# edin-dal/sdqlpy

Measured on AMD Instinct MI355X. Metric: tpch_q1_q3_q5_sf10_rows_per_sec, higher is better.
Workload: dtype f64; 1 GPU; TPCH Q1+Q3+Q5 SF=10 per GPU (BASELINE metric: Q1/Q3/Q5 at SF=10; q1 = configs[1], q3 = configs[2]); partitioning=none

## Files before the change

### sdqlpy_amd/csrc/sdqh_hip.hip

```cpp
#include <hip/hip_runtime.h>

#include <algorithm>
#include <atomic>
#include <chrono>
#include <cmath>
#include <cstdio>
#include <cstdlib>
#include <cstring>
#include <string>
#include <thread>
#include <type_traits>
#include <map>
#include <vector>

#include "sdqh_host.hpp"

using namespace sdqh_host;

static int ensure_index(sdqh_ctx* ctx, sdqh_table* tb);

namespace sdqh_host {

int fail(sdqh_ctx* ctx, int code, const std::string& msg) {
    if (ctx) ctx->err = msg;
// ... 620 lines not shown
    const std::string n(name);
    if (n == "resident_cap" && value >= 1 && value <= 8) ctx->opt_resident_cap = (int)value;
    else if (n == "async_copies" && (value == 0 || value == 1)) ctx->opt_async_copies = (int)value;
    else if (n == "resident_stream" && value >= 1 && value <= 8) ctx->opt_resident_stream = (int)value;
    else if (n == "probe_chunk" && value >= 1 && value <= 64) ctx->opt_probe_chunk = (int)value;
    else if (n == "probe_unroll" && (value == 1 || value == 2 || value == 4)) ctx->opt_probe_unroll = (int)value;
    else if (n == "stage_batch" && (value == 2 || value == 4 || value == 8)) ctx->opt_stage_batch = (int)value;
    else if (n == "stage_eager" && (value == 0 || value == 1)) ctx->opt_stage_eager = (int)value;
    else if (n == "stage_eager_pay" && (value == 0 || value == 1)) ctx->opt_stage_eager_pay = (int)value;
    else if (n == "stage_waves_per_cu" && value >= 4 && value <= 64) ctx->opt_stage_waves_per_cu = (int)value;
    else if (n == "direct_index" && (value == 0 || value == 1)) ctx->opt_direct_index = (int)value;
    else if (n == "row_pack" && (value == 0 || value == 1)) ctx->opt_row_pack = (int)value;
    else if (n == "cluster_pack" && value >= 0 && value <= 2) ctx->opt_cluster_pack = (int)value;
    else if (n == "cluster_list" && (value == 0 || value == 1)) ctx->opt_cluster_list = (int)value;
    else if (n == "x_driven" && value >= 0 && value <= (1 << 20)) ctx->opt_x_driven = (int)value;
    else if (n == "delta8" && (value == 0 || value == 1)) ctx->opt_delta8 = (int)value;
    else if (n == "word_pairs" && (value == 0 || value == 1)) ctx->opt_word_pairs = (int)value;
    else if (n == "coarse_kb" && value >= 0 && value <= 96) ctx->opt_coarse_kb = (int)value;
    else if (n == "lookup_pipeline" && value >= -1 && value <= 1) ctx->opt_lookup_pipeline = (int)value;
    else if (n == "probe_pipeline" && value >= 0 && value <= 1) ctx->opt_probe_pipeline = (int)value;
    else if (n == "lookup_debug") ctx->opt_lookup_debug = (int)value;
    else if (n == "fuse_small" && value >= 0 && value <= 1) ctx->opt_fuse_small = (int)value;
    else if (n == "lds_key_set" && value >= 0 && value <= 1) ctx->opt_lds_key_set = (int)value;
    else if (n == "fill_ahead" && value >= 0 && value <= 1) { ctx->opt_fill_ahead = (int)value; for (auto& b : ctx->pool) b.nhabits = 0; }
    else if (n == "str_rows" && (value == 0 || value == 32 || value == 64)) ctx->opt_str_rows = (int)value;
    else if (n == "rank_increasing" && value >= 0 && value <= 1) ctx->opt_rank_increasing = (int)value;
    else if (n == "feature_min_rows" && value >= 0) ctx->opt_feature_min_rows = value;
    else if (n == "narrow" && value >= 0 && value <= 1) ctx->opt_narrow = (int)value;
    else if (n == "tight" && value >= 0 && value <= 1) ctx->opt_tight = (int)value;
    else if (n == "spin_sync" && value >= 0 && value <= 1) ctx->opt_spin_sync = (int)value;
// ... 1964 lines not shown
```

### sdqlpy_amd/csrc/sdqh_host.hpp

```cpp
#pragma once
#include <hip/hip_runtime.h>

#include <atomic>
#include <map>
#include <string>
#include <vector>

#include "sdqh.h"
#include "sdqh_kernels.hpp"

namespace sdqh_host {

struct FillHabit { size_t off, bytes; int byte; bool clean; };
struct PoolBlock {
    void* ptr; size_t size; bool free;
    FillHabit habits[4] = {};
    int nhabits = 0;
    uint64_t alloc_seq = 0;
    bool fill_use = false;
    const void* graph_owner = nullptr;
};
struct ProfEntry { const char* name; hipEvent_t e0, e1; double ms; int64_t model_bytes; };

constexpr size_t STAGING_BYTES = 32u << 20;
// ... 65 lines not shown
    int opt_tight = 1;
    hipStream_t side[2] = {nullptr, nullptr};
    hipEvent_t side_ev[4] = {nullptr, nullptr, nullptr, nullptr};
    int opt_side_streams = 1;
    int opt_side_priority = 1;
    int opt_copy_kernel = 0;
    int opt_copy_nt = 1;
    int opt_row_index = 1;
    int opt_grouped_index = 1;
    int opt_grouped_pairs = 1;
    int opt_index_inline = 1;
    int opt_lane_int = 1;
    int opt_lane_resident = 2;
    int opt_window = 0;
    int opt_x_driven = 64;
    int opt_word_pairs = 0;
    int opt_delta8 = 1;
    int opt_x_waves = 0;
    void* rs_dev[2] = {nullptr, nullptr}; size_t rs_bytes[2] = {0, 0};
    hipEvent_t rs_copied[2] = {nullptr, nullptr}; bool rs_used[2] = {false, false};
    int rs_cur = 0; bool rs_pending = false;
    hipEvent_t rs_ready = nullptr;
    volatile uint32_t* sync_flag = nullptr; uint32_t sync_seq = 0; int opt_spin_sync = 1;
    int opt_async_result = 1;
    int opt_narrow = 1;
    int opt_stage_pipeline = 0;
    int opt_span_index = 1;
    int opt_dense_increasing = 1;
    int opt_probe_pipeline = 0;
    const void* coarse_stat_col = nullptr; uint64_t* coarse_stat = nullptr;
// ... 136 lines not shown
```

### sdqlpy_amd/csrc/sdqh_x.hip

```cpp
#define SDQH_DECLS_ONLY 1
#include <hip/hip_runtime.h>
#include <hip/hiprtc.h>

#include <dlfcn.h>
#include <sys/stat.h>
#include <unistd.h>

#include <algorithm>
#include <chrono>
#include <cstdio>
#include <cstdlib>
#include <cstring>
#include <fstream>
#include <mutex>
#include <sstream>
#include <string>
#include <vector>

#include "sdqh_host.hpp"
#include "sdqh_xkernels.hpp"

using namespace sdqh_host;

namespace {
// ... 43 lines not shown
    int cmp_kind[SDQH_MAX_XOPS];
    int cmp_col[SDQH_MAX_XOPS];
    uint32_t cc[X_MAX_CONST]; int ncc = 0;
    bool affine[SDQH_MAX_XCOLS] = {};
    int64_t dlo[SDQH_MAX_XCOLS] = {};
    signed char irange[SDQH_MAX_XOPS] = {};
    bool fake = false;
    bool vstage = false; int nlk = 0; int lk_op[2] = {-1, -1};
    bool pref32 = false;
    int ival = -1;
    bool pnear = false;
    bool pwin = false;
    bool phash = false;
    bool want_driven = false;
    bool driven = false; int driven_col = -1;
    uint32_t gather32 = 0;
    mutable uint32_t lay[SDQH_MAX_XTABLES] = {};
    std::vector<char> scope;
};

bool op_is_light(const sdqh_xop& o) {
    switch (o.code) {
        case SDQH_X_LOOKUP: case SDQH_X_FIELD: case SDQH_X_ACC: case SDQH_X_STR: case SDQH_X_STRIDX: case SDQH_X_CHAR: case SDQH_X_RUNNEW: return false;
        default: return true;
    }
}
void closure(const sdqh_program* p, int k, std::vector<char>& seen) {
    if (k < 0 || k >= p->nops || seen[(size_t)k]) return;
    seen[(size_t)k] = 1;
    const sdqh_xop& o = p->ops[k];
// ... 293 lines not shown
    if (!twin) return nullptr;
    uint32_t* ridx = static_cast<uint32_t*>(attach_alloc(ctx, c, ((size_t)range + 1) * 4 + 64));
    if (!ridx) return nullptr;
    const int64_t nvals = (int64_t)range + 1;
    const unsigned grid = (unsigned)std::max<int64_t>(1, std::min<int64_t>((nvals + 255) / 256, (int64_t)ctx->num_cu * 16));
    { KernelScope ks(ctx, "k_run_index"); hipLaunchKernelGGL(k_run_index, dim3(grid), dim3(256), 0, ctx->stream, twin, c->nrows, c->mn, nvals, ridx); }
    if (hipGetLastError() != hipSuccess || hipStreamSynchronize(ctx->stream) != hipSuccess) { (void)hipGetLastError(); attach_free(ctx, c, ridx); return nullptr; }
    c->run_index = ridx; c->run_index_state = 1;
    return ridx;
}

void tight_plan(sdqh_ctx* ctx, int64_t nrows, XInfo* x) {
    const sdqh_program* p = x->p;
    for (int k = 0; k < p->nops; ++k) x->cmp_cc[k] = x->cmp_kind[k] = x->cmp_col[k] = -1;
    for (int c = 0; c < SDQH_MAX_XCOLS; ++c) { x->enc[c] = ENC_RAW; x->dict_slot[c] = -1; }
    x->tight = false; x->nd = 0; x->ncc = 0; x->gather32 = 0; x->pref32 = false; x->pnear = false; x->pwin = false; x->driven = false; x->driven_col = -1; x->phash = false;
    const bool fake = ctx->compile_only && std::getenv("SDQLPY_AMD_FAKE_CODES") != nullptr;
    static const std::vector<int64_t> fake_dict = {0, 1, 2, 3};
    const bool regs_all = x->direct || x->vstage;
    if (!ctx->opt_tight || x->ncols < 1 || (!regs_all && x->scols.empty())) return;
    x->tight = true;
    x->fake = fake;
    uint32_t text_twins = 0;
    for (int c = 0; c < x->ncols; ++c) if (x->cols[c]->dtype == SDQH_STR) text_twins |= x->narrow_mask & (1u << c);
    x->narrow_mask = text_twins;
    x->scope.assign((size_t)p->nops, regs_all ? 1 : 0);
    std::vector<char> streamed((size_t)x->ncols, regs_all ? 1 : 0);
    if (!regs_all) {
        for (int g = 0; g < x->nstream_gates; ++g) closure(p, p->gates[g], x->scope);
        if (x->prefilter_part0 >= 0) closure(p, x->prefilter_part0, x->scope);
        for (int c : x->scols) streamed[(size_t)c] = 1;
// ... 68 lines not shown
    if (fake && !regs_all && x->prefilter_op >= 0 && !x->prefilter_composite) x->pref32 = true;
    static const bool xdebug = std::getenv("SDQLPY_AMD_X_DEBUG") != nullptr;
    if (xdebug && !regs_all && x->prefilter_op >= 0) {
        const sdqh_table* t = x->tabs[x->tab_of[x->prefilter_op]];
        std::fprintf(stderr, "[x] prefilter: composite %d bm %p shift %d lin_rb %lld range [%lld, %lld] irange %d pref32 %d gates %d rows %lld\n", (int)x->prefilter_composite, (const void*)t->dev.bm,
                     (int)t->dev.bm_shift, (long long)t->dev.lin_rb, (long long)t->dev.bm_lo, (long long)t->dev.bm_hi, (int)x->irange[x->prefilter_part0], (int)x->pref32, x->nstream_gates, (long long)nrows);
    }
    if (x->pref32) {
        const sdqh_xop& ko = p->ops[x->prefilter_part0];
        x->pnear = fake ? true : (ko.code == SDQH_X_COL && column_span8(ctx, const_cast<sdqh_column*>(ko.col)));
        x->pwin = fake ? std::getenv("SDQLPY_AMD_FAKE_WINDOW") != nullptr : (ctx->opt_window != 0 && x->pnear);
        if (!fake && x->want_driven && ctx->opt_x_driven > 0 && x->nstream_gates == 0 && ko.code == SDQH_X_COL) {
            const int c = x->col_of[x->prefilter_part0];
            sdqh_column* kc = const_cast<sdqh_column*>(x->cols[c]);
            if (kc->dtype == SDQH_I64 && kc->nrows == nrows && nrows < ((int64_t)1 << 31) && column_run_index(ctx, kc)) { x->driven = true; x->driven_col = c; }
            if (xdebug) std::fprintf(stderr, "[x] driven walk: enc %d column rows %lld run index %d -> %d\n", x->enc[c], (long long)kc->nrows, kc->run_index_state, (int)x->driven);
        }
    }
    if (!regs_all && !fake && !x->vstage && ctx->opt_delta8 && x->pref32 && !x->driven) {
        const sdqh_xop& ko = p->ops[x->prefilter_part0];
        if (ko.code == SDQH_X_COL) {
            const int c = x->col_of[x->prefilter_part0];
            sdqh_column* kc = const_cast<sdqh_column*>(x->cols[c]);
            if (x->enc[c] == ENC_N32 && kc->nrows == nrows && x->pnear && column_delta8(ctx, kc)) { x->enc[c] = ENC_D8; x->narrow_mask &= ~(1u << c); x->gather32 |= 1u << c; }
        }
    }
    if (x->vstage && !fake && ctx->opt_delta8) {
        for (int c = 0; c < x->ncols; ++c) {
            sdqh_column* kc = const_cast<sdqh_column*>(x->cols[c]);
            if (x->enc[c] == ENC_N32 && kc->dtype == SDQH_I64 && kc->nrows == nrows && column_span8(ctx, kc) && column_delta8(ctx, kc)) { x->enc[c] = ENC_D8; x->narrow_mask &= ~(1u << c); }
// ... 101 lines not shown
                }
                case ENC_D8: return "(int64_t)xt_d8(" + w + ", i)";
                case ENC_N32: return o.type == SDQH_T_F64 ? "narrow_decode(xt_i32(" + w + ", i))" : "(int64_t)xt_i32(" + w + ", i)";
                case ENC_RAW: return o.type == SDQH_T_F64 ? "x_f(xt_i64(" + w + ", i))" : "xt_i64(" + w + ", i)";
                default: return "0 /* a 16-bit code has no value form */";
            }
        }
        if (mode == 1) raw = "(H == 0 ? s[" + std::to_string(slot_of[(size_t)c]) + "].x : s[" + std::to_string(slot_of[(size_t)c]) + "].y)";
        else raw = "s[" + std::to_string(slot_of[(size_t)c]) + "]." + half;
        return o.type == SDQH_T_F64 ? "x_f(" + raw + ")" : raw;
    }
    std::string i64_at(int c, const std::string& at) const {
        if (((x.gather32 | x.narrow_mask) >> c) & 1u) return "(int64_t)static_cast<const int32_t*>(a.ncol[" + std::to_string(c) + "])[" + at + "]";
        return "static_cast<const int64_t*>(a.col[" + std::to_string(c) + "])[" + at + "]";
    }
    void emit(int k) {
        if (k < 0 || done[(size_t)k]) return;
        const sdqh_xop& o = x.p->ops[k];
        auto v = [](int j) { return "v" + std::to_string(j); };
        const std::string K = std::to_string(k);
        std::string e;
        if (mode == 3 && !(is_cmp(o.code) && x.cmp_cc[k] >= 0)) {
            const int c = single_col(k);
            const bool bare = o.code == SDQH_X_COL;
            if (c >= 0 && (int)tabs.size() < (bare ? MAX_TABS : MAX_DERIVED)) {
                if (tab_of[(size_t)k] < 0) { tab_of[(size_t)k] = (int)tabs.size(); tabs.push_back({k, c}); }
                const std::string cell = "tab[" + std::to_string(tab_of[(size_t)k]) + "][xt_u8(s.c" + std::to_string(slot_of[(size_t)c]) + ", i)]";
                e = o.type == SDQH_T_F64 ? "x_f(" + cell + ")" : o.type == SDQH_T_BOOL ? "(" + cell + " != 0)" : cell;
                os << "        const " << ctype(o.type) << " v" << K << " = " << e << ";\n";
                if (o.code == SDQH_X_SELECT) os << "        const bool b" << K << " = false;\n";
                done[(size_t)k] = 1;
                return;
            }
        }
        switch (o.code) {
            case SDQH_X_COL: e = col_expr(k); break;
            case SDQH_X_ROWID: e = mode == 0 ? row : "r"; break;
            case SDQH_X_CONST:
                e = o.type == SDQH_T_F64 ? "a.cf[" + std::to_string(x.const_of[k]) + "]" : (o.type == SDQH_T_BOOL ? "(a.ci[" + std::to_string(x.const_of[k]) + "] != 0)" : "a.ci[" + std::to_string(x.const_of[k]) + "]");
                break;
            case SDQH_X_LOOKUP:
                emit(o.a);
                os << "        const uint32_t e" << K << " = x_lookup_l<" << lay_lit(x.tab_of[k]) << ">(a.tab[" << x.tab_of[k] << "], " << v(o.a) << ", " << bad(o.a) << ");\n";
                e = "(e" + K + " != NO_ROW)";
                break;
            case SDQH_X_FIELD:
                emit(o.a);
                e = "x_field(a.tab[" + std::to_string(x.tab_of[o.a]) + "], " + std::to_string(o.aux) + ", e" + std::to_string(o.a) + ")";
                if (o.type == SDQH_T_F64) e = "x_f(" + e + ")";
                break;
            case SDQH_X_ACC:
                emit(o.a);
                e = o.aux < 0 ? "x_hits_l<" + lay_lit(x.tab_of[o.a]) + ">(a.tab[" + std::to_string(x.tab_of[o.a]) + "], e" + std::to_string(o.a) + ")"
                              : "x_acc_l<" + lay_lit(x.tab_of[o.a]) + ">(a.tab[" + std::to_string(x.tab_of[o.a]) + "], " + std::to_string(o.aux) + ", e" + std::to_string(o.a) + ")";
                break;
            case SDQH_X_ADD: case SDQH_X_SUB: case SDQH_X_MUL: {
                emit(o.a); emit(o.b);
                const char* sym = o.code == SDQH_X_ADD ? " + " : o.code == SDQH_X_SUB ? " - " : " * ";
                if (mode == 3 && o.type == SDQH_T_I64 && x.irange[k] >= 1 && x.irange[o.a] >= 1 && x.irange[o.b] >= 1) {
                    if (o.code == SDQH_X_MUL && x.irange[o.a] == 2 && x.irange[o.b] == 2) e = "(int64_t)__mul24((int)" + v(o.a) + ", (int)" + v(o.b) + ")";
                    else e = "(int64_t)((int32_t)" + v(o.a) + sym + "(int32_t)" + v(o.b) + ")";
                } else e = "(" + v(o.a) + sym + v(o.b) + ")";
                break;
            }
            case SDQH_X_DIV: emit(o.a); emit(o.b); e = "(" + v(o.a) + " / " + v(o.b) + ")"; break;
            case SDQH_X_NEG: emit(o.a); e = "(-" + v(o.a) + ")"; break;
            case SDQH_X_I2F: emit(o.a); e = "(double)" + v(o.a); break;
            case SDQH_X_YEAR: emit(o.a); e = "(" + v(o.a) + " / 10000)"; break;
            case SDQH_X_DIVI: case SDQH_X_MODI:
// ... 227 lines not shown
    out << "    __device__ __forceinline__ static const uint32_t* lkbm(const XArgs& a, int l) { return ";
    if (x.nlk == 0) out << "nullptr";
    else if (x.nlk == 1) out << "a.tab[" << x.tab_of[x.lk_op[0]] << "].bm";
    else out << "l == 0 ? a.tab[" << x.tab_of[x.lk_op[0]] << "].bm : a.tab[" << x.tab_of[x.lk_op[1]] << "].bm";
    out << "; }\n";
    out << "    __device__ __forceinline__ static void row(const XArgs& a, const Regs& s, const int64_t (*tab)[256], const int i, const int64_t r, XOut<NV>& o) {\n" << row << "    }\n};\n";
    out << "extern \"C\" __global__ __launch_bounds__(256) void " << VSTAGE_ENTRY << "(XArgs a, XStage<P::NV>::Args s, int64_t nrows, int64_t seg_rows, int nseg) {\n";
    out << "    x_vstage8<P>(a, s, nrows, seg_rows, nseg);\n}\n";
    return out.str();
}

std::string generate(const XInfo& x, Sink sink, bool direct) {
    if (x.vstage && sink == SINK_STAGE) return generate_vstage(x);
    if (x.tight && direct) return generate_tight(x, sink);
    const bool q8 = x.tight && !direct;
    const sdqh_program* p = x.p;
    Gen g(x);
    std::vector<int> scols = x.scols;
    int first_gate = x.nstream_gates;
    if (direct) { scols.clear(); for (int c = 0; c < x.ncols; ++c) scols.push_back(c); first_gate = 0; }
    for (size_t i = 0; i < scols.size(); ++i) g.slot_of[(size_t)scols[i]] = (int)i;
    const int ns = (int)scols.size(), nsx = std::max(1, ns);
    std::ostringstream out;
    out << "#include \"sdqh_xkernels.hpp\"\nusing namespace sdqh;\n";
    std::vector<int> tcols, twidth; std::vector<std::vector<int>> tops;
    bool stage_text = !direct;
    for (int k = 0; k < p->nops && stage_text; ++k) {
        const int code = p->ops[k].code;
        if (code != SDQH_X_STR && code != SDQH_X_STRIDX && code != SDQH_X_CHAR) continue;
        const int c = x.col_of[k], w = p->ops[k].col ? p->ops[k].col->width : 0;
// ... 83 lines not shown
        out << "    __device__ __forceinline__ static bool stest(const XArgs& a, const Regs& s, const int64_t (*tab)[256], const int i) {\n" << stest8 << "    }\n";
        out << "    __device__ __forceinline__ static bool spre(const XArgs& a, const Regs& s, const int64_t (*tab)[256], const int i, uint32_t& widx, uint32_t& bit) {\n" << spre8 << "    }\n";
        out << "    static constexpr bool PREF32 = " << ((x.pref32 || x.phash) ? "true" : "false") << ", PWIN = " << (x.pwin ? "true" : "false") << ";\n";
        out << "    __device__ __forceinline__ static bool spre32(const XArgs& a, const Regs& s, const int64_t (*tab)[256], const int i, uint32_t& off) {\n"
            << ((x.pref32 || x.phash) ? spre32 : std::string("        off = 0; return false;\n")) << "    }\n";
        if (x.phash) {
            out << "    static constexpr bool PHASH = true;\n";
            out << "    __device__ __forceinline__ static const TableHeader* shdr(const XArgs& a) { return a.tab[" << x.tab_of[x.prefilter_op] << "].hdr; }\n";
            out << "    __device__ __forceinline__ static const uint32_t* sbitmap(const XArgs& a) { return a.tab[" << x.tab_of[x.prefilter_op] << "].hf; }\n";
        } else
        out << "    __device__ __forceinline__ static const uint32_t* sbitmap(const XArgs& a) { return "
            << (x.prefilter_op >= 0 ? "x_prefilter_bitmap(a.tab[" + std::to_string(x.tab_of[x.prefilter_op]) + "], " + (x.prefilter_composite ? "true" : "false") + ")" : std::string("nullptr")) << "; }\n";
        if (x.driven && sink == SINK_GROUP) {
            out << "    static constexpr bool DRIVEN = true;\n";
            out << "    __device__ __forceinline__ static const DevTable& dtab(const XArgs& a) { return a.tab[" << x.tab_of[x.prefilter_op] << "]; }\n";
        }
    }
    if (!tcols.empty()) {
        out << "    __device__ __forceinline__ static constexpr int scol(int j) { return j == 0 ? " << tcols[0] << " : " << (tcols.size() > 1 ? tcols[1] : tcols[0]) << "; }\n";
        out << "    __device__ __forceinline__ static constexpr int swidth(int j) { return j == 0 ? " << twidth[0] << " : " << (twidth.size() > 1 ? twidth[1] : twidth[0]) << "; }\n";
        auto tb = [&](size_t j) { return ((x.narrow_mask >> tcols[j]) & 1u) != 0; };
        out << "    __device__ __forceinline__ static constexpr bool sbytes(int j) { return j == 0 ? " << (tb(0) ? "true" : "false") << " : " << (tb(tcols.size() > 1 ? 1 : 0) ? "true" : "false") << "; }\n";
        out << "    template <int J> __device__ __forceinline__ static void sops(const XArgs& a, const uint32_t* region, int off, int64_t (&sres)[" << nsopx << "]) {\n";
        for (size_t j = 0; j < tcols.size(); ++j) {
            out << "        if constexpr (J == " << j << ") {\n";
            if (!tb(j)) out << "            const uint32_t* f = region + (off >> 2);\n";
            for (int k : tops[j]) out << "            sres[" << g.sres_of[(size_t)k] << "] = (int64_t)" << (tb(j) ? g.text_op(k, "region, off, " + std::to_string(twidth[j]), true, true) : g.text_op(k, "f, " + std::to_string(twidth[j]), true)) << ";\n";
            out << "        }\n";
        }
        out << "    }\n";
// ... 9 lines not shown
    out << "    __device__ __forceinline__ static void stest(const XArgs& a, const Pair<int64_t> (&s)[" << nsx << "], bool& p0, bool& p1) {\n";
    if (!direct) for (int h = 0; h < 2; ++h) {
        g.reset(); g.mode = 2; g.half = h ? "y" : "x"; g.os.str("");
        out << "      {\n";
        for (int q = 0; q < x.nstream_gates; ++q) { g.emit(p->gates[q]); g.os << "        p" << h << " = p" << h << " && v" << p->gates[q] << ";\n"; }
        if (x.prefilter_op >= 0) {
            g.emit(x.prefilter_part0);
            g.os << "        p" << h << " = p" << h << " && x_may_hit(a.tab[" << x.tab_of[x.prefilter_op] << "], v" << x.prefilter_part0 << ", " << (x.prefilter_composite ? "true" : "false") << ");\n";
        }
        out << g.os.str() << "      }\n";
    }
    out << "    }\n";
    }
    auto body = [&](int mode, int from_gate) {
        g.reset(); g.mode = mode; g.os.str("");
        static const bool no_levels = std::getenv("SDQLPY_AMD_X_NOLEVELS") != nullptr;
        g.pinning = mode == 0 && !no_levels;
        g.want.assign((size_t)p->nops, 0);
        if (g.pinning) {
            for (int q = from_gate; q < p->ngates; ++q) closure(p, p->gates[q], g.want);
            for (int k = 0; k < p->nops; ++k) if (g.want[(size_t)k] && p->ops[k].code == SDQH_X_COL && g.is_row_load(k)) g.emit(k);
            g.flush_pins();
        }
        for (int q = from_gate; q < p->ngates; ++q) { g.emit(p->gates[q]); g.flush_pins(); g.os << "        if (!v" << p->gates[q] << ") return false;\n"; }
        if (g.pinning) {
            std::vector<char> rest((size_t)p->nops, 0);
            if (p->key >= 0) closure(p, p->key, rest);
            for (int v = 0; v < p->nvals; ++v) closure(p, p->vals[v], rest);
            if (x.probe_op >= 0) closure(p, x.probe_op, rest);
            g.want = rest;
            for (int k = 0; k < p->nops; ++k) if (rest[(size_t)k] && p->ops[k].code == SDQH_X_LOOKUP) g.emit(k);
            g.flush_pins();
            for (int k = 0; k < p->nops; ++k) if (rest[(size_t)k] && g.is_row_load(k)) g.emit(k);
            g.flush_pins();
        }
        if (p->key >= 0) { g.emit(p->key); g.os << "        o.key = v" << p->key << "; o.bad = " << g.bad(p->key) << ";\n"; }
        else g.os << "        o.key = 0; o.bad = false;\n";
        for (int v = 0; v < p->nvals; ++v) {
            g.emit(p->vals[v]);
            g.os << "        o.val[" << v << "] = " << (p->ops[p->vals[v]].type == SDQH_T_F64 ? "x_bits(v" + std::to_string(p->vals[v]) + ")" : "v" + std::to_string(p->vals[v])) << ";\n";
        }
        if (x.probe_op >= 0) { g.emit(x.probe_op); g.os << "        o.ent = e" << x.probe_op << ";\n"; } else g.os << "        o.ent = NO_ROW;\n";
        g.os << "        return true;\n";
        return g.os.str();
    };
    out << "    template <int H> __device__ __forceinline__ static bool eval_regs(const XArgs& a, const Pair<int64_t> (&s)[" << nsx << "], int64_t r, XOut<NV>& o) {\n";
    if (direct) out << body(1, 0); else out << "        return false;\n";
    out << "    }\n";
    out << "    __device__ __forceinline__ static bool eval_row(const XArgs& a, int64_t r, const int64_t (&sres)[" << nsopx << "], XOut<NV>& o) {\n";
    if (!direct) out << body(0, first_gate); else out << "        return false;\n";
    out << "    }\n};\n";
    const std::string sn = sink_name(sink);
    out << "extern \"C\" __global__ __launch_bounds__(256) void " << entry_name(sink, direct, q8) << "(XArgs a, " << sn << "<P::NV>::Args s, int64_t nrows, int64_t seg_rows, int nseg) {\n";
    if (direct) out << "    x_direct<P, " << sn << ">(a, s, nrows);\n";
    else out << "    " << (q8 ? "x_queue8" : "x_queue") << "<P, " << sn << ", " << (sink == SINK_STAGE ? "true" : "false") << ">(a, s, nrows, seg_rows, nseg);\n";
    out << "}\n";
    return out.str();
}

struct JitState {
    std::mutex mu;
    bool headers_loaded = false; std::string h_abi, h_kernels, h_xkernels, src_dir, cache_dir, why_unusable;
    std::map<std::string, hipFunction_t> kernels;
    int64_t compiled = 0, from_disk = 0;
// ... 29 lines not shown
        J.why_unusable = "run-time specialisation needs sdqh_kernels.hpp, sdqh_xkernels.hpp next to libsdqlhip.so and include/sdqh.h (looked in " + dir + ")";
        return false;
    }
    if (const char* env = std::getenv("SDQLPY_AMD_JIT_CACHE")) J.cache_dir = env;
    else J.cache_dir = dir + "/../jit_cache";
    (void)mkdir(J.cache_dir.c_str(), 0777);
    return true;
}

uint64_t structure_hash(const XInfo& x, Sink sink, bool direct) {
    const sdqh_program* p = x.p;
    uint64_t h = 1469598103934665603ull;
    auto mix = [&](uint64_t v) { h ^= v; h *= 0x9E3779B97F4A7C15ull; h ^= h >> 29; };
    mix((uint64_t)sink * 2 + (direct ? 1 : 0)); mix((uint64_t)x.narrow_mask);
    if (x.tight) {
        mix(0x7167ull); mix((uint64_t)x.gather32); mix((x.pref32 ? 1ull : 0ull) | (x.vstage ? 2ull : 0ull) | (x.pwin ? 4ull : 0ull) | (x.pnear ? 8ull : 0ull) | (x.driven ? 16ull : 0ull) | (x.phash ? 32ull : 0ull) | ((uint64_t)(x.ival + 1) << 8));
        for (int c = 0; c < x.ncols; ++c) mix(((uint64_t)(uint32_t)x.enc[c] << 32) | ((uint32_t)(x.affine[c] ? 1 : 0) << 16) | (uint32_t)(x.dict_slot[c] & 0xFFFF));
        for (int k = 0; k < x.p->nops; ++k) mix((uint64_t)(uint8_t)x.irange[k]);
        for (int k = 0; k < x.p->nops; ++k) mix(((uint64_t)(uint32_t)x.cmp_cc[k] << 32) | ((uint32_t)x.cmp_kind[k] << 8) | (uint32_t)(x.cmp_col[k] & 0xFF));
    } mix((uint64_t)p->nops); mix((uint64_t)(int64_t)p->key); mix((uint64_t)(int64_t)x.probe_op);
    for (int k = 0; k < p->nops; ++k) {
        const sdqh_xop& o = p->ops[k];
        mix(((uint64_t)(uint32_t)o.code << 32) | (uint32_t)o.type); mix(((uint64_t)(uint32_t)o.a << 32) | (uint32_t)o.b); mix(((uint64_t)(uint32_t)o.c << 32) | (uint32_t)o.aux);
        mix(((uint64_t)(uint32_t)x.col_of[k] << 32) | (uint32_t)x.tab_of[k]); mix(((uint64_t)(uint32_t)x.const_of[k] << 32) | (uint32_t)x.str_off[k]);
        if (o.code == SDQH_X_DIVI || o.code == SDQH_X_MODI) mix((uint64_t)o.imm_i);
        if (o.code == SDQH_X_STR || o.code == SDQH_X_STRIDX) { mix((uint64_t)o.slen); for (int i = 0; i < o.slen; ++i) mix(o.str[i]); }
        if (o.code == SDQH_X_STR || o.code == SDQH_X_STRIDX || o.code == SDQH_X_CHAR) mix((uint64_t)(o.col ? o.col->width : 0));
    }
    mix((uint64_t)p->ngates); for (int g = 0; g < p->ngates; ++g) mix((uint64_t)p->gates[g]);
    mix((uint64_t)p->nvals); for (int v = 0; v < p->nvals; ++v) mix((uint64_t)p->vals[v]);
    return h;
// ... 673 lines not shown
```

### sdqlpy_amd/csrc/sdqh_xkernels.hpp

```cpp
#pragma once
#include "sdqh_kernels.hpp"

#ifndef XGL_IVAL
#define XGL_IVAL -1
#endif
#ifndef XE_EXP
#define XE_EXP 0
#endif
#ifndef X8_DRAIN_AT
#define X8_DRAIN_AT WAVE
#endif
#ifndef X8_EXP
#define X8_EXP 0
#endif
#ifndef X8_EXP_MINROWS
#define X8_EXP_MINROWS 0
#endif
#ifndef X8_EXP_BUILD
#define X8_EXP_BUILD 0
#endif
#ifndef X8_PIPE
#define X8_PIPE 0
#endif
#ifndef XV_MASKED
// ... 25 lines not shown
    uint32_t cc[X_MAX_CONST];
    int64_t dlo[SDQH_MAX_XCOLS];
    DevTable tab[SDQH_MAX_XTABLES];
    int64_t ci[X_MAX_CONST];
    double cf[X_MAX_CONST];
    uint32_t spool[SDQH_MAX_XSTR];
    int32_t* flags;
    int64_t key_lo, key_hi;
    const uint32_t* run_index;
    int64_t run_lo, run_hi;
    int32_t driven_ratio, _pad_driven;
};
template <class...> using x_void_t = void;
template <class P, class = void> struct x_is_driven { static constexpr bool value = false; };
template <class P> struct x_is_driven<P, x_void_t<decltype(P::DRIVEN)>> { static constexpr bool value = P::DRIVEN; };
template <class P, class = void> struct x_is_phash { static constexpr bool value = false; };
template <class P> struct x_is_phash<P, x_void_t<decltype(P::PHASH)>> { static constexpr bool value = P::PHASH; };

template <int NV> struct XOut {
    int64_t key;
    int64_t val[NV > 0 ? NV : 1];
    uint32_t ent;
    bool bad;
};

__device__ __forceinline__ double x_f(int64_t bits) { return __longlong_as_double(bits); }
__device__ __forceinline__ int64_t x_bits(double v) { return __double_as_longlong(v); }

template <bool TAIL> __device__ __forceinline__ Pair<int64_t> x_sload_narrow_i(const void* p, int64_t r, int64_t nrows) {
    return loadc<TAIL, true>(static_cast<const int64_t*>(p), r, nrows);
// ... 838 lines not shown
    total = __shfl(incl, WAVE - 1, WAVE);
    return incl - v;
}
__device__ __forceinline__ int wave_excl_prefix4(uint32_t v, int& total) {
    int below = 0, all = 0;
#pragma unroll
    for (int k = 0; k < 4; ++k) {
        const uint64_t b = __ballot((v >> k) & 1u);
        below += (int)__builtin_amdgcn_mbcnt_hi((uint32_t)(b >> 32), __builtin_amdgcn_mbcnt_lo((uint32_t)b, 0u)) << k;
        all += __popcll(b) << k;
    }
    total = all;
    return below;
}

template <class Sink> __device__ __forceinline__ constexpr bool x_exp_on() { return X8_EXP_BUILD ? !Sink::FINAL : Sink::FINAL; }
template <class P, template <int> class SinkT, bool SEGMENTED>
__device__ __forceinline__ void x_queue8(const XArgs& a, const typename SinkT<P::NV>::Args& sa, int64_t nrows, int64_t seg_rows, int nseg) {
    using Sink = SinkT<P::NV>;
    __shared__ int32_t s_row[TPB / WAVE][X8_CAP];
    __shared__ uint32_t s_text[P::NSC > 0 ? TPB / WAVE : 1][P::NSC > 0 ? XSTR_UNITS : 1];
    __shared__ int64_t s_tab[P::ND > 0 ? P::ND : 1][256];
    P::load_dicts(a, s_tab);
    Sink sink;
    sink.init(sa);
    __syncthreads();
    const int seg = blockIdx.x * (TPB / WAVE) + threadIdx.x / WAVE;
    const bool live = seg < nseg;
    int32_t* q_row = s_row[threadIdx.x / WAVE];
    uint32_t* s_str = s_text[P::NSC > 0 ? threadIdx.x / WAVE : 0];
    const int lane = lane_id();
    constexpr int64_t STEP2 = (int64_t)X8_STEP * X8_U;
    const bool tiled = !SEGMENTED && seg_rows == 0;
    const int64_t whole_end = tiled ? nrows / STEP2 * STEP2 : 0;
    const int64_t stride = tiled ? (int64_t)nseg * STEP2 : STEP2;
    int phase = tiled ? 1 : 0;
    const int64_t begin = tiled ? 0 : (int64_t)seg * seg_rows;
    int64_t end = tiled ? whole_end : begin + seg_rows; if (end > nrows) end = nrows;
    if constexpr (SEGMENTED) sink.begin_segment(begin);
    int qn = 0;
    const uint32_t* pbm = P::sbitmap(a);
    uint32_t hmask = 0;
    if constexpr (x_is_phash<P>::value) hmask = hf_mask_of(P::shdr(a)->cap_mask);
    auto drain = [&](int first, int count) {
        XOut<P::NV> o;
        int64_t sres[P::NSOP > 0 ? P::NSOP : 1] = {0};
        if constexpr (P::NSC > 0) x_stage_text<P, 0>(a, q_row, begin, first, count, s_str, sres);
        if constexpr (P::NSC > 1) x_stage_text<P, 1>(a, q_row, begin, first, count, s_str, sres);
        bool pass = false; int64_t r = 0;
        if (lane < count) { r = begin + (int64_t)q_row[first + lane]; pass = P::eval_row(a, r, sres, o); }
        if constexpr (X8_EXP == 4 && x_exp_on<Sink>()) {
            if (lane < count) { XOut<P::NV> o2; const bool p2 = P::eval_row(a, r ^ 1, sres, o2); pass = pass && (p2 || (uint32_t)a.key_hi != 0x12345678u); }
        }
        if constexpr (X8_EXP == 14 && x_exp_on<Sink>()) pass = pass && (o.key == -12345 || nrows < (int64_t)X8_EXP_MINROWS);
        if constexpr ((X8_EXP == 5 || X8_EXP == 10) && x_exp_on<Sink>()) { int pi = pass ? 1 : 0; asm volatile("" : "+v"(pi)); pass = pi != 0 && (uint32_t)a.key_hi == 0x12345678u; }
        sink.consume(a, sa, pass, r, o);
    };
    auto enqueue8 = [&](int64_t r0, uint32_t m) {
        if (!__ballot(m != 0)) return;
        int total;
        int at = qn + wave_excl_prefix4(__popc(m), total);
        const int32_t off = (int32_t)(r0 - begin);
        while (m) { q_row[at++] = off + (__ffs((int)m) - 1); m &= m - 1u; }
        qn += total;
    };
    bool driven = false;
    uint64_t d_nq = 0, d_q = 0, d_nwords = 0;
    XWindow d_w = {0u, 0u, 0u, 0u};
    uint32_t d_bit0 = 0, d_cur = 0, d_end = 0;
    auto d_quad = [&](uint64_t q) {
        const uint64_t wb = q * 4;
        if (wb + 4 <= d_nwords) return x_load_window(pbm + wb);
        XWindow v = {0u, 0u, 0u, 0u};
        if (wb < d_nwords) v.x = pbm[wb];
        if (wb + 1 < d_nwords) v.y = pbm[wb + 1];
        if (wb + 2 < d_nwords) v.z = pbm[wb + 2];
        return v;
    };
    if constexpr (x_is_driven<P>::value) {
        if (live && tiled && pbm && a.run_index && a.driven_ratio > 0) {
            const DevTable& t = P::dtab(a);
            d_nwords = ((uint64_t)(t.bm_hi - t.bm_lo) + 32) >> 5;
            d_nq = (d_nwords + 3) >> 2;
            const uint64_t ns = d_nq < (uint64_t)WAVE ? d_nq : (uint64_t)WAVE;
            int bits = 0, tot = 0;
            if ((uint64_t)lane < ns) { const XWindow v = d_quad((uint64_t)lane * (d_nq / ns)); bits = __popc(v.x) + __popc(v.y) + __popc(v.z) + __popc(v.w); }
            (void)wave_excl_prefix(bits, tot);
            const double est = ns ? (double)tot * ((double)d_nq / (double)ns) : 0.0;
            driven = est * (double)a.driven_ratio <= (double)nrows;
            d_q = (uint64_t)seg * WAVE;
        }
    }
    if (live) {
#if X8_PIPE
        typename P::Regs pre[X8_U];
        {
            const int64_t b0 = tiled ? (int64_t)seg * STEP2 : begin;
            if (b0 + STEP2 <= end) {
#pragma unroll
                for (int u = 0; u < X8_U; ++u) P::template sload<false>(a, b0 + (int64_t)u * X8_STEP + (int64_t)lane * XT_R, nrows, pre[u]);
            }
        }
#endif
        for (int64_t b = tiled ? (int64_t)seg * STEP2 : begin;;) {
// ... 5 lines not shown
                        if (d_q >= d_nq) last = true;
                        else {
                            const uint64_t q = d_q + (uint64_t)lane;
                            d_w = q < d_nq ? d_quad(q) : XWindow{0u, 0u, 0u, 0u};
                            d_bit0 = (uint32_t)(q * 128);
                            d_q += (uint64_t)nseg * WAVE;
                        }
                    }
                    if (!last) {
                        if (d_cur >= d_end && (d_w.x | d_w.y | d_w.z | d_w.w) != 0u) {
                            const int j = d_w.x ? 0 : d_w.y ? 1 : d_w.z ? 2 : 3;
                            const uint32_t word = j == 0 ? d_w.x : j == 1 ? d_w.y : j == 2 ? d_w.z : d_w.w;
                            const uint32_t bp = (uint32_t)__ffs((int)word) - 1u, rest = word & (word - 1u);
                            if (j == 0) d_w.x = rest; else if (j == 1) d_w.y = rest; else if (j == 2) d_w.z = rest; else d_w.w = rest;
                            const int64_t key = P::dtab(a).bm_lo + (int64_t)(d_bit0 + (uint32_t)j * 32u + bp);
                            if (key >= a.run_lo && key <= a.run_hi) { d_cur = a.run_index[key - a.run_lo]; d_end = a.run_index[key - a.run_lo + 1]; }
                        }
                        const uint32_t n = d_end - d_cur < 8u ? d_end - d_cur : 8u;
                        const int64_t r0 = (int64_t)d_cur;
                        d_cur += n;
                        enqueue8(r0, (1u << n) - 1u);
                    }
                }
            }
            if (!produced) {
            if (phase == 1 && b >= end) {
                phase = 2;
                if (seg == 0) { b = whole_end; end = nrows; }
            }
            last = b >= end;
            if (last) {
            } else if (b + (int64_t)X8_STEP * X8_U <= end) {
                typename P::Regs s[X8_U];
#if X8_PIPE
#pragma unroll
                for (int u = 0; u < X8_U; ++u) s[u] = pre[u];
// ... 134 lines not shown
                for (int i = 0; i < XT_R; ++i) m |= (r0 + i < end && P::stest(a, s1, s_tab, i)) ? (1u << i) : 0u;
                enqueue8(r0, m);
                b += X8_STEP;
            }
            }
            int head = 0;
            if constexpr (X8_EXP == 3 && x_exp_on<Sink>()) { if ((uint32_t)a.key_hi != 0x12345678u && nrows >= (int64_t)X8_EXP_MINROWS) qn = 0; }
            while (qn - head >= X8_DRAIN_AT || (last && qn > head)) {
                const int n = qn - head >= WAVE ? WAVE : qn - head;
                drain(head, n);
                head += n;
            }
            if (last) break;
            if (head) {
                const int left = qn - head;
                int32_t keepv = 0;
                if (lane < left) keepv = q_row[head + lane];
                if (lane < left) q_row[lane] = keepv;
                qn = left;
            }
        }
        if constexpr (SEGMENTED) sink.end_segment(sa, seg, begin);
    }
    sink.finish(a, sa);
}



constexpr int XV_CAP = 64 + X8_STEP;
template <bool Q32> struct XQueueWord { using type = int64_t; };
template <> struct XQueueWord<true> { using type = int32_t; };
template <class P>
__device__ __forceinline__ void x_vstage8(const XArgs& a, const typename XStage<P::NV>::Args& sa, int64_t nrows, int64_t seg_rows, int nseg) {
// ... 221 lines not shown
```

Measured before the change: 439.1 billion rows/s.

## Carry driven-walk hash entry through queue to skip per-row gate lookup

In the driven walk path, the hash-table entry for each key is looked up once when the walker reaches a new key run. That entry is then stored in a shared-memory side queue next to the row offsets. The generated eval_row takes a known flag and the entry, so it can read fields directly instead of redoing the prefilter lookup for every row. This adds a second LDS queue, which enlarges shared memory and may cut occupancy. It also adds a lookup per key in the walker and a scalarized driven flag.

```diff
diff --git a/sdqlpy_amd/csrc/sdqh_hip.hip b/sdqlpy_amd/csrc/sdqh_hip.hip
--- a/sdqlpy_amd/csrc/sdqh_hip.hip
+++ b/sdqlpy_amd/csrc/sdqh_hip.hip
@@ -658,6 +658,7 @@
     else if (n == "cluster_pack" && value >= 0 && value <= 2) ctx->opt_cluster_pack = (int)value;
     else if (n == "cluster_list" && (value == 0 || value == 1)) ctx->opt_cluster_list = (int)value;
     else if (n == "x_driven" && value >= 0 && value <= (1 << 20)) ctx->opt_x_driven = (int)value;
+    else if (n == "walk_entry" && value >= 0 && value <= 1) ctx->opt_walk_entry = (int)value;
     else if (n == "delta8" && (value == 0 || value == 1)) ctx->opt_delta8 = (int)value;
     else if (n == "word_pairs" && (value == 0 || value == 1)) ctx->opt_word_pairs = (int)value;
     else if (n == "coarse_kb" && value >= 0 && value <= 96) ctx->opt_coarse_kb = (int)value;
diff --git a/sdqlpy_amd/csrc/sdqh_host.hpp b/sdqlpy_amd/csrc/sdqh_host.hpp
--- a/sdqlpy_amd/csrc/sdqh_host.hpp
+++ b/sdqlpy_amd/csrc/sdqh_host.hpp
@@ -103,6 +103,7 @@
     int opt_lane_resident = 2;
     int opt_window = 0;
     int opt_x_driven = 64;
+    int opt_walk_entry = 1;
     int opt_word_pairs = 0;
     int opt_delta8 = 1;
     int opt_x_waves = 0;
diff --git a/sdqlpy_amd/csrc/sdqh_x.hip b/sdqlpy_amd/csrc/sdqh_x.hip
--- a/sdqlpy_amd/csrc/sdqh_x.hip
+++ b/sdqlpy_amd/csrc/sdqh_x.hip
@@ -81,6 +81,7 @@
     bool phash = false;
     bool want_driven = false;
     bool driven = false; int driven_col = -1;
+    bool walk_entry = false;
     uint32_t gather32 = 0;
     mutable uint32_t lay[SDQH_MAX_XTABLES] = {};
     std::vector<char> scope;
@@ -404,7 +405,7 @@
     const sdqh_program* p = x->p;
     for (int k = 0; k < p->nops; ++k) x->cmp_cc[k] = x->cmp_kind[k] = x->cmp_col[k] = -1;
     for (int c = 0; c < SDQH_MAX_XCOLS; ++c) { x->enc[c] = ENC_RAW; x->dict_slot[c] = -1; }
-    x->tight = false; x->nd = 0; x->ncc = 0; x->gather32 = 0; x->pref32 = false; x->pnear = false; x->pwin = false; x->driven = false; x->driven_col = -1; x->phash = false;
+    x->tight = false; x->nd = 0; x->ncc = 0; x->gather32 = 0; x->pref32 = false; x->pnear = false; x->pwin = false; x->driven = false; x->driven_col = -1; x->walk_entry = false; x->phash = false;
     const bool fake = ctx->compile_only && std::getenv("SDQLPY_AMD_FAKE_CODES") != nullptr;
     static const std::vector<int64_t> fake_dict = {0, 1, 2, 3};
     const bool regs_all = x->direct || x->vstage;
@@ -503,6 +504,7 @@
             const int c = x->col_of[x->prefilter_part0];
             sdqh_column* kc = const_cast<sdqh_column*>(x->cols[c]);
             if (kc->dtype == SDQH_I64 && kc->nrows == nrows && nrows < ((int64_t)1 << 31) && column_run_index(ctx, kc)) { x->driven = true; x->driven_col = c; }
+            x->walk_entry = x->driven && ctx->opt_walk_entry != 0 && p->ngates > 0 && p->gates[0] == x->prefilter_op && p->ops[x->prefilter_op].a == x->prefilter_part0;
             if (xdebug) std::fprintf(stderr, "[x] driven walk: enc %d column rows %lld run index %d -> %d\n", x->enc[c], (long long)kc->nrows, kc->run_index_state, (int)x->driven);
         }
     }
@@ -634,6 +636,53 @@
         if (((x.gather32 | x.narrow_mask) >> c) & 1u) return "(int64_t)static_cast<const int32_t*>(a.ncol[" + std::to_string(c) + "])[" + at + "]";
         return "static_cast<const int64_t*>(a.col[" + std::to_string(c) + "])[" + at + "]";
     }
+    std::string entry_expr(int k) const {
+        const sdqh_xop& o = x.p->ops[k];
+        const std::string t = std::to_string(x.tab_of[o.a]), ent = "e" + std::to_string(o.a);
+        if (o.code == SDQH_X_FIELD) {
+            const std::string e = "x_field(a.tab[" + t + "], " + std::to_string(o.aux) + ", " + ent + ")";
+            return o.type == SDQH_T_F64 ? "x_f(" + e + ")" : e;
+        }
+        return o.aux < 0 ? "x_hits_l<" + lay_lit(x.tab_of[o.a]) + ">(a.tab[" + t + "], " + ent + ")"
+                         : "x_acc_l<" + lay_lit(x.tab_of[o.a]) + ">(a.tab[" + t + "], " + std::to_string(o.aux) + ", " + ent + ")";
+    }
+    void emit_walked_gate(int kl) {
+        const sdqh_program* p = x.p;
+        const int ka = p->ops[kl].a;
+        bool shared = p->key == ka;
+        for (int v = 0; v < p->nvals; ++v) shared = shared || p->vals[v] == ka;
+        for (int q = 0; q < p->ngates; ++q) shared = shared || p->gates[q] == ka;
+        for (int j = 0; j < p->nops; ++j) {
+            const sdqh_xop& u = p->ops[j];
+            if (j == kl || u.code == SDQH_X_COL || u.code == SDQH_X_CONST || u.code == SDQH_X_ROWID) continue;
+            shared = shared || u.a == ka || u.b == ka || (u.code == SDQH_X_SELECT && u.c == ka);
+        }
+        const std::string K = std::to_string(kl), A = std::to_string(ka);
+        for (int k = 0; k < p->nops; ++k) if (k != ka && want[(size_t)k] && p->ops[k].code == SDQH_X_COL && is_row_load(k)) emit(k);
+        if (shared) emit(ka);
+        else { os << "        int64_t v" << A << " = 0;\n        if (!known) v" << A << " = " << col_expr(ka) << ";\n"; done[(size_t)ka] = 1; }
+        const std::vector<std::string> cols = pins;
+        std::vector<int> fields;
+        for (int j = kl + 1; j < p->nops; ++j) {
+            const sdqh_xop& f = p->ops[j];
+            if ((f.code == SDQH_X_FIELD || f.code == SDQH_X_ACC) && f.a == kl && want[(size_t)j]) fields.push_back(j);
+        }
+        os << "        uint32_t e" << K << " = ek;\n";
+        for (int j : fields) os << "        " << ctype(p->ops[j].type) << " v" << j << " = 0;\n";
+        os << "        if (known) {\n";
+        for (int j : fields) { os << "            v" << j << " = " << entry_expr(j) << ";\n"; pins.push_back("v" + std::to_string(j)); }
+        flush_pins();
+        os << "        } else {\n";
+        pins = shared ? std::vector<std::string>() : std::vector<std::string>{"v" + A};
+        pins.insert(pins.begin(), cols.begin(), cols.end());
+        flush_pins();
+        os << "            e" << K << " = x_lookup_l<" << lay_lit(x.tab_of[kl]) << ">(a.tab[" << x.tab_of[kl] << "], v" << A << ", false);\n";
+        for (int j : fields) { os << "            v" << j << " = " << entry_expr(j) << ";\n"; pins.push_back("v" + std::to_string(j)); }
+        flush_pins();
+        os << "        }\n        const bool v" << K << " = (e" << K << " != NO_ROW);\n";
+        done[(size_t)kl] = 1;
+        for (int j : fields) done[(size_t)j] = 1;
+    }
     void emit(int k) {
         if (k < 0 || done[(size_t)k]) return;
         const sdqh_xop& o = x.p->ops[k];
@@ -664,15 +713,9 @@
                 os << "        const uint32_t e" << K << " = x_lookup_l<" << lay_lit(x.tab_of[k]) << ">(a.tab[" << x.tab_of[k] << "], " << v(o.a) << ", " << bad(o.a) << ");\n";
                 e = "(e" + K + " != NO_ROW)";
                 break;
-            case SDQH_X_FIELD:
+            case SDQH_X_FIELD: case SDQH_X_ACC:
                 emit(o.a);
-                e = "x_field(a.tab[" + std::to_string(x.tab_of[o.a]) + "], " + std::to_string(o.aux) + ", e" + std::to_string(o.a) + ")";
-                if (o.type == SDQH_T_F64) e = "x_f(" + e + ")";
-                break;
-            case SDQH_X_ACC:
-                emit(o.a);
-                e = o.aux < 0 ? "x_hits_l<" + lay_lit(x.tab_of[o.a]) + ">(a.tab[" + std::to_string(x.tab_of[o.a]) + "], e" + std::to_string(o.a) + ")"
-                              : "x_acc_l<" + lay_lit(x.tab_of[o.a]) + ">(a.tab[" + std::to_string(x.tab_of[o.a]) + "], " + std::to_string(o.aux) + ", e" + std::to_string(o.a) + ")";
+                e = entry_expr(k);
                 break;
             case SDQH_X_ADD: case SDQH_X_SUB: case SDQH_X_MUL: {
                 emit(o.a); emit(o.b);
@@ -930,6 +973,8 @@
     if (x.vstage && sink == SINK_STAGE) return generate_vstage(x);
     if (x.tight && direct) return generate_tight(x, sink);
     const bool q8 = x.tight && !direct;
+    static const bool no_levels = std::getenv("SDQLPY_AMD_X_NOLEVELS") != nullptr;
+    const bool walked = q8 && x.driven && x.walk_entry && sink == SINK_GROUP && !no_levels && x.nstream_gates == 0;
     const sdqh_program* p = x.p;
     Gen g(x);
     std::vector<int> scols = x.scols;
@@ -1043,6 +1088,7 @@
         if (x.driven && sink == SINK_GROUP) {
             out << "    static constexpr bool DRIVEN = true;\n";
             out << "    __device__ __forceinline__ static const DevTable& dtab(const XArgs& a) { return a.tab[" << x.tab_of[x.prefilter_op] << "]; }\n";
+            if (walked) out << "    __device__ __forceinline__ static uint32_t dentry(const XArgs& a, int64_t key) { return x_lookup_l<" << g.lay_lit(x.tab_of[x.prefilter_op]) << ">(a.tab[" << x.tab_of[x.prefilter_op] << "], key, false); }\n";
         }
     }
     if (!tcols.empty()) {
@@ -1082,12 +1128,12 @@
     }
     auto body = [&](int mode, int from_gate) {
         g.reset(); g.mode = mode; g.os.str("");
-        static const bool no_levels = std::getenv("SDQLPY_AMD_X_NOLEVELS") != nullptr;
         g.pinning = mode == 0 && !no_levels;
         g.want.assign((size_t)p->nops, 0);
         if (g.pinning) {
             for (int q = from_gate; q < p->ngates; ++q) closure(p, p->gates[q], g.want);
-            for (int k = 0; k < p->nops; ++k) if (g.want[(size_t)k] && p->ops[k].code == SDQH_X_COL && g.is_row_load(k)) g.emit(k);
+            if (walked && mode == 0) g.emit_walked_gate(x.prefilter_op);
+            else for (int k = 0; k < p->nops; ++k) if (g.want[(size_t)k] && p->ops[k].code == SDQH_X_COL && g.is_row_load(k)) g.emit(k);
             g.flush_pins();
         }
         for (int q = from_gate; q < p->ngates; ++q) { g.emit(p->gates[q]); g.flush_pins(); g.os << "        if (!v" << p->gates[q] << ") return false;\n"; }
@@ -1115,7 +1161,7 @@
     out << "    template <int H> __device__ __forceinline__ static bool eval_regs(const XArgs& a, const Pair<int64_t> (&s)[" << nsx << "], int64_t r, XOut<NV>& o) {\n";
     if (direct) out << body(1, 0); else out << "        return false;\n";
     out << "    }\n";
-    out << "    __device__ __forceinline__ static bool eval_row(const XArgs& a, int64_t r, const int64_t (&sres)[" << nsopx << "], XOut<NV>& o) {\n";
+    out << "    __device__ __forceinline__ static bool eval_row(const XArgs& a, int64_t r, const int64_t (&sres)[" << nsopx << "], XOut<NV>& o" << (walked ? ", const bool known, uint32_t ek" : "") << ") {\n";
     if (!direct) out << body(0, first_gate); else out << "        return false;\n";
     out << "    }\n};\n";
     const std::string sn = sink_name(sink);
@@ -1175,7 +1221,7 @@
     auto mix = [&](uint64_t v) { h ^= v; h *= 0x9E3779B97F4A7C15ull; h ^= h >> 29; };
     mix((uint64_t)sink * 2 + (direct ? 1 : 0)); mix((uint64_t)x.narrow_mask);
     if (x.tight) {
-        mix(0x7167ull); mix((uint64_t)x.gather32); mix((x.pref32 ? 1ull : 0ull) | (x.vstage ? 2ull : 0ull) | (x.pwin ? 4ull : 0ull) | (x.pnear ? 8ull : 0ull) | (x.driven ? 16ull : 0ull) | (x.phash ? 32ull : 0ull) | ((uint64_t)(x.ival + 1) << 8));
+        mix(0x7167ull); mix((uint64_t)x.gather32); mix((x.pref32 ? 1ull : 0ull) | (x.vstage ? 2ull : 0ull) | (x.pwin ? 4ull : 0ull) | (x.pnear ? 8ull : 0ull) | (x.driven ? 16ull : 0ull) | (x.phash ? 32ull : 0ull) | (x.walk_entry ? 64ull : 0ull) | ((uint64_t)(x.ival + 1) << 8));
         for (int c = 0; c < x.ncols; ++c) mix(((uint64_t)(uint32_t)x.enc[c] << 32) | ((uint32_t)(x.affine[c] ? 1 : 0) << 16) | (uint32_t)(x.dict_slot[c] & 0xFFFF));
         for (int k = 0; k < x.p->nops; ++k) mix((uint64_t)(uint8_t)x.irange[k]);
         for (int k = 0; k < x.p->nops; ++k) mix(((uint64_t)(uint32_t)x.cmp_cc[k] << 32) | ((uint32_t)x.cmp_kind[k] << 8) | (uint32_t)(x.cmp_col[k] & 0xFF));
diff --git a/sdqlpy_amd/csrc/sdqh_xkernels.hpp b/sdqlpy_amd/csrc/sdqh_xkernels.hpp
--- a/sdqlpy_amd/csrc/sdqh_xkernels.hpp
+++ b/sdqlpy_amd/csrc/sdqh_xkernels.hpp
@@ -63,6 +63,8 @@
 template <class...> using x_void_t = void;
 template <class P, class = void> struct x_is_driven { static constexpr bool value = false; };
 template <class P> struct x_is_driven<P, x_void_t<decltype(P::DRIVEN)>> { static constexpr bool value = P::DRIVEN; };
+template <class P, class = void> struct x_has_dentry { static constexpr bool value = false; };
+template <class P> struct x_has_dentry<P, x_void_t<decltype(&P::dentry)>> { static constexpr bool value = x_is_driven<P>::value; };
 template <class P, class = void> struct x_is_phash { static constexpr bool value = false; };
 template <class P> struct x_is_phash<P, x_void_t<decltype(P::PHASH)>> { static constexpr bool value = P::PHASH; };
 
@@ -931,11 +933,18 @@
     return below;
 }
 
+template <class P, int NSOPX> __device__ __forceinline__ bool x_eval_row(const XArgs& a, int64_t r, const int64_t (&sres)[NSOPX], XOut<P::NV>& o, bool known, uint32_t ek) {
+    if constexpr (x_has_dentry<P>::value) return P::eval_row(a, r, sres, o, known, ek);
+    else return P::eval_row(a, r, sres, o);
+}
+constexpr int X8_DCAP = X8_DRAIN_AT + X8_STEP;
+template <class P> constexpr int x8_cap() { return x_has_dentry<P>::value && 2 * X8_DCAP > X8_CAP ? 2 * X8_DCAP : X8_CAP; }
 template <class Sink> __device__ __forceinline__ constexpr bool x_exp_on() { return X8_EXP_BUILD ? !Sink::FINAL : Sink::FINAL; }
 template <class P, template <int> class SinkT, bool SEGMENTED>
 __device__ __forceinline__ void x_queue8(const XArgs& a, const typename SinkT<P::NV>::Args& sa, int64_t nrows, int64_t seg_rows, int nseg) {
     using Sink = SinkT<P::NV>;
-    __shared__ int32_t s_row[TPB / WAVE][X8_CAP];
+    constexpr bool WALKED = x_has_dentry<P>::value;
+    __shared__ int32_t s_row[TPB / WAVE][x8_cap<P>()];
     __shared__ uint32_t s_text[P::NSC > 0 ? TPB / WAVE : 1][P::NSC > 0 ? XSTR_UNITS : 1];
     __shared__ int64_t s_tab[P::ND > 0 ? P::ND : 1][256];
     P::load_dicts(a, s_tab);
@@ -945,6 +954,7 @@
     const int seg = blockIdx.x * (TPB / WAVE) + threadIdx.x / WAVE;
     const bool live = seg < nseg;
     int32_t* q_row = s_row[threadIdx.x / WAVE];
+    uint32_t* q_ent = reinterpret_cast<uint32_t*>(q_row) + (WALKED ? X8_DCAP : 0);
     uint32_t* s_str = s_text[P::NSC > 0 ? threadIdx.x / WAVE : 0];
     const int lane = lane_id();
     constexpr int64_t STEP2 = (int64_t)X8_STEP * X8_U;
@@ -957,6 +967,7 @@
     if constexpr (SEGMENTED) sink.begin_segment(begin);
     int qn = 0;
     const uint32_t* pbm = P::sbitmap(a);
+    bool driven = false;
     uint32_t hmask = 0;
     if constexpr (x_is_phash<P>::value) hmask = hf_mask_of(P::shdr(a)->cap_mask);
     auto drain = [&](int first, int count) {
@@ -965,9 +976,14 @@
         if constexpr (P::NSC > 0) x_stage_text<P, 0>(a, q_row, begin, first, count, s_str, sres);
         if constexpr (P::NSC > 1) x_stage_text<P, 1>(a, q_row, begin, first, count, s_str, sres);
         bool pass = false; int64_t r = 0;
-        if (lane < count) { r = begin + (int64_t)q_row[first + lane]; pass = P::eval_row(a, r, sres, o); }
+        if (lane < count) {
+            r = begin + (int64_t)q_row[first + lane];
+            uint32_t ek = NO_ROW;
+            if constexpr (WALKED) { if (driven) ek = q_ent[first + lane]; }
+            pass = x_eval_row<P>(a, r, sres, o, driven, ek);
+        }
         if constexpr (X8_EXP == 4 && x_exp_on<Sink>()) {
-            if (lane < count) { XOut<P::NV> o2; const bool p2 = P::eval_row(a, r ^ 1, sres, o2); pass = pass && (p2 || (uint32_t)a.key_hi != 0x12345678u); }
+            if (lane < count) { XOut<P::NV> o2; const bool p2 = x_eval_row<P>(a, r ^ 1, sres, o2, false, NO_ROW); pass = pass && (p2 || (uint32_t)a.key_hi != 0x12345678u); }
         }
         if constexpr (X8_EXP == 14 && x_exp_on<Sink>()) pass = pass && (o.key == -12345 || nrows < (int64_t)X8_EXP_MINROWS);
         if constexpr ((X8_EXP == 5 || X8_EXP == 10) && x_exp_on<Sink>()) { int pi = pass ? 1 : 0; asm volatile("" : "+v"(pi)); pass = pi != 0 && (uint32_t)a.key_hi == 0x12345678u; }
@@ -981,10 +997,17 @@
         while (m) { q_row[at++] = off + (__ffs((int)m) - 1); m &= m - 1u; }
         qn += total;
     };
-    bool driven = false;
     uint64_t d_nq = 0, d_q = 0, d_nwords = 0;
     XWindow d_w = {0u, 0u, 0u, 0u};
-    uint32_t d_bit0 = 0, d_cur = 0, d_end = 0;
+    uint32_t d_bit0 = 0, d_cur = 0, d_end = 0, d_ent = NO_ROW;
+    auto enqueue8e = [&](int64_t r0, uint32_t n, uint32_t ent) {
+        if (!__ballot(n != 0)) return;
+        int total;
+        int at = qn + wave_excl_prefix4(n, total);
+        const int32_t off = (int32_t)(r0 - begin);
+        for (uint32_t i = 0; i < n; ++i) { q_row[at + (int)i] = off + (int32_t)i; q_ent[at + (int)i] = ent; }
+        qn += total;
+    };
     auto d_quad = [&](uint64_t q) {
         const uint64_t wb = q * 4;
         if (wb + 4 <= d_nwords) return x_load_window(pbm + wb);
@@ -1005,6 +1028,7 @@
             (void)wave_excl_prefix(bits, tot);
             const double est = ns ? (double)tot * ((double)d_nq / (double)ns) : 0.0;
             driven = est * (double)a.driven_ratio <= (double)nrows;
+            if constexpr (WALKED) driven = __builtin_amdgcn_readfirstlane((int)driven) != 0;
             d_q = (uint64_t)seg * WAVE;
         }
     }
@@ -1040,12 +1064,15 @@
                             const uint32_t bp = (uint32_t)__ffs((int)word) - 1u, rest = word & (word - 1u);
                             if (j == 0) d_w.x = rest; else if (j == 1) d_w.y = rest; else if (j == 2) d_w.z = rest; else d_w.w = rest;
                             const int64_t key = P::dtab(a).bm_lo + (int64_t)(d_bit0 + (uint32_t)j * 32u + bp);
-                            if (key >= a.run_lo && key <= a.run_hi) { d_cur = a.run_index[key - a.run_lo]; d_end = a.run_index[key - a.run_lo + 1]; }
+                            if (key >= a.run_lo && key <= a.run_hi) {
+                                if constexpr (WALKED) d_ent = P::dentry(a, key);
+                                d_cur = a.run_index[key - a.run_lo]; d_end = a.run_index[key - a.run_lo + 1];
+                            }
                         }
                         const uint32_t n = d_end - d_cur < 8u ? d_end - d_cur : 8u;
                         const int64_t r0 = (int64_t)d_cur;
                         d_cur += n;
-                        enqueue8(r0, (1u << n) - 1u);
+                        if constexpr (WALKED) enqueue8e(r0, n, d_ent); else enqueue8(r0, (1u << n) - 1u);
                     }
                 }
             }
@@ -1210,9 +1237,11 @@
             if (last) break;
             if (head) {
                 const int left = qn - head;
-                int32_t keepv = 0;
+                int32_t keepv = 0; uint32_t keepe = 0;
                 if (lane < left) keepv = q_row[head + lane];
+                if constexpr (WALKED) { if (driven && lane < left) keepe = q_ent[head + lane]; }
                 if (lane < left) q_row[lane] = keepv;
+                if constexpr (WALKED) { if (driven && lane < left) q_ent[lane] = keepe; }
                 qn = left;
             }
         }
```

After: 438.5 billion rows/s. No clear change (-0.1%).
